# marco-wojtek/Exploring-MuZero-on-DOG

Hardware: AMD Instinct MI355X
Metric: self-play env steps/sec + MCTS sims/sec, det-MADN batch=4096, 1/2/4/8 GPU (higher is better)
Workload: dtype f32

## Files before the change

### exploring-muzero-on-dog_amd/csrc/launch.hpp

```cpp
#pragma once
#include "common.hpp"

namespace muz {

constexpr int kMaxSims = 100;
constexpr int kMaxNodes = kMaxSims + 1;
constexpr int kMaxDepth = 64;
static inline int check_search_limits(int num_simulations, int max_depth) {
  const bool ok = num_simulations >= 1 && num_simulations <= kMaxSims && max_depth >= 1 && max_depth <= kMaxDepth;
  return ok ? MUZ_OK : MUZ_E_UNSUPPORTED;
}
static inline int check_search_call(int num_simulations, int max_depth, int n, const void* root_logits,
                                    const void* root_value, const void* root_embedding, const void* legal_bits,
                                    const void* workspace, int64_t workspace_bytes, int64_t (*need)(int, int),
                                    const void* action, const void* action_weights, const void* root_value_out) {
  if (check_search_limits(num_simulations, max_depth)) return MUZ_E_UNSUPPORTED;
  MUZ_HOST_CHECK(n >= 0 && root_logits && root_value && root_embedding && legal_bits && workspace && action &&
                 action_weights && root_value_out);
  MUZ_HOST_CHECK(workspace_bytes >= need(n, num_simulations));
  return MUZ_OK;
}

static inline bool ring_scalar_base() {
  const char* e = getenv("MUZ_RING_ADDR");
  return !e || atoi(e) != 0;
}

struct SearchArgs {
  int S, D, max_considered;
  float value_scale, maxvisit_init, gumbel_scale;
  unsigned long long seed;
  int turn;
  const int32_t* key_game = nullptr;
  const int32_t* key_turn = nullptr;
  int exact_select = 0;
  int games_per_wg = 8;
};
static inline SearchArgs make_search_args(const muz_search_cfg& cfg) {
  SearchArgs sa;
  sa.S = cfg.num_simulations;
  sa.D = cfg.max_depth;
  sa.max_considered = cfg.max_num_considered;
  sa.value_scale = cfg.value_scale;
  sa.maxvisit_init = cfg.maxvisit_init;
  sa.gumbel_scale = cfg.gumbel_scale;
  sa.seed = cfg.seed;
  sa.turn = cfg.turn;
  return sa;
}

int launch_root_inference(const muz_net_w& w, const float* obs, int n, const int* n_dev, float* conv_scratch,
                          float* logits, float* value, float* emb, hipStream_t s, int32_t* host_counts = nullptr);

int launch_root_inference(const muz_classic_net_w& w, const float* obs, int n, const int* n_dev, float* conv_scratch,
                          float* logits, float* value, float* emb, hipStream_t s);

int launch_repr_conv(const muz_repr_w& r, const float* obs, int C, int n, const int* n_dev, float* conv,
                     hipStream_t s, int32_t* host_counts = nullptr);
int launch_dense0(const muz_dense& d0, int n, const int* n_dev, float* conv, hipStream_t s);
int launch_film(const muz_dyn_w& d, int A, hipStream_t s);

int launch_gumbel_search(const muz_net_w& w, const SearchArgs& sa, const float* root_logits, const float* root_value,
                         const float* root_emb, const uint32_t* legal, const float* gumbel, const int32_t* game_id,
                         int n, const int* n_dev, void* workspace, int32_t* action, float* weights, float* value,
                         hipStream_t s);

int64_t search_workspace_bytes(int n, int S);

struct PuctArgs {
  int S, D, qtransform;
  float min_value, max_value, dir_frac, dir_alpha, pb_c_init, pb_c_base, temperature;
  unsigned long long seed;
  int turn;
  const int32_t* key_game = nullptr;
  const int32_t* key_turn = nullptr;
};
template <class Cfg>
static inline PuctArgs puct_args_of(const Cfg& cfg, int qtransform, float min_value, float max_value) {
  PuctArgs pa;
  pa.S = cfg.num_simulations;
  pa.D = cfg.max_depth;
  pa.qtransform = qtransform;
  pa.min_value = min_value;
  pa.max_value = max_value;
  pa.dir_frac = cfg.dirichlet_fraction;
  pa.dir_alpha = cfg.dirichlet_alpha;
  pa.pb_c_init = cfg.pb_c_init;
  pa.pb_c_base = cfg.pb_c_base;
  pa.temperature = cfg.temperature;
  pa.seed = cfg.seed;
  pa.turn = cfg.turn;
  return pa;
}
static inline PuctArgs make_puct_args(const muz_puct_cfg& cfg) {
  return puct_args_of(cfg, cfg.qtransform, cfg.min_value, cfg.max_value);
}
static inline PuctArgs make_puct_args(const muz_stoch_cfg& cfg) {
  return puct_args_of(cfg, MUZ_QT_PARENT_SIBLINGS, -1.f, 1.f);
}
static inline int check_puct_cfg(const muz_puct_cfg& cfg) {
  if (cfg.qtransform != MUZ_QT_MIN_MAX && cfg.qtransform != MUZ_QT_PARENT_SIBLINGS) return MUZ_E_UNSUPPORTED;
  if (!(cfg.max_value > cfg.min_value)) return MUZ_E_UNSUPPORTED;
  if (!(cfg.dirichlet_fraction >= 0.f && cfg.dirichlet_fraction <= 1.f)) return MUZ_E_UNSUPPORTED;
  if (!(cfg.dirichlet_alpha > 0.f) || !(cfg.pb_c_base > 0.f) || !(cfg.temperature >= 0.f)) return MUZ_E_UNSUPPORTED;
  return MUZ_OK;
}
static inline int check_stoch_cfg(const muz_stoch_cfg& cfg) {
  if (!(cfg.dirichlet_fraction >= 0.f && cfg.dirichlet_fraction <= 1.f)) return MUZ_E_UNSUPPORTED;
  if (!(cfg.dirichlet_alpha > 0.f) || !(cfg.pb_c_base > 0.f) || !(cfg.temperature >= 0.f)) return MUZ_E_UNSUPPORTED;
  if (!(cfg.pb_c_init == cfg.pb_c_init)) return MUZ_E_UNSUPPORTED;
  return MUZ_OK;
}
int launch_puct_search(const muz_net_w& w, const PuctArgs& pa, const float* root_logits, const float* root_value,
                       const float* root_emb, const uint32_t* legal, const float* dirichlet, const float* gumbel,
                       const int32_t* game_id, int n, const int* n_dev, void* workspace, int32_t* action,
                       float* weights, float* value, hipStream_t s);

struct SArgs {
  int S, D, A;
  float dir_frac, dir_alpha, pb_c_init, pb_c_base, temperature;
  unsigned long long seed;
  int turn;
  const int32_t* key_game = nullptr;
  const int32_t* key_turn = nullptr;
};
SArgs make_sargs(const muz_stoch_cfg& cfg, int A);
int launch_stochastic_search(const muz_classic_net_w& w, const SArgs& sa, const float* root_logits,
                             const float* root_value, const float* root_emb, const uint32_t* legal,
                             const float* dirichlet, const float* gumbel, const int32_t* game_id, int n, const int* n_dev,
                             void* workspace, int32_t* action, float* weights, float* value, hipStream_t s);
int64_t stochastic_workspace_bytes(int n, int S);
int check_classic_net(const muz_classic_net_w* w);

}
```

### exploring-muzero-on-dog_amd/csrc/nets.hip

```cpp
#include <type_traits>

#include "launch.hpp"
#include "nn.hpp"

namespace muz {

constexpr int kConvRowsPad = 64;
constexpr int kPreLd = 64 + 4;
#ifndef MUZ_CONV_PAD
#define MUZ_CONV_PAD 8
#endif
constexpr int kC1Ld = 32 + MUZ_CONV_PAD;
constexpr int kC2Ld = 64 + MUZ_CONV_PAD;

template <int N, int LDO>
__device__ __forceinline__ void ln_positions(const float* pre, float* out, int out_row0, const AS4 muz_ln& P) {
  const int pos = threadIdx.x >> 2, q = threadIdx.x & 3;
  if (pos >= 56) return;
  constexpr int PER = N / 4;
  float v[PER], s = 0.f, s2 = 0.f;
#pragma unroll
  for (int i = 0; i < PER; ++i) {
    v[i] = pre[pos * kPreLd + q + 4 * i];
    s += v[i];
    s2 = fmaf(v[i], v[i], s2);
  }
  s += dpp<DPP_XOR1>(s);
  s += dpp<DPP_XOR2>(s);
  s2 += dpp<DPP_XOR1>(s2);
  s2 += dpp<DPP_XOR2>(s2);
  const float mean = s / (float)N, mean2 = s2 / (float)N;
  const float inv = ln_rstd(fmaxf(0.f, fmaf(-mean, mean, mean2)) + 1e-6f);
#pragma unroll
  for (int i = 0; i < PER; ++i) {
    const int c = q + 4 * i;
    out[(out_row0 + pos) * LDO + c] = fmaxf(fmaf(v[i] - mean, inv * gp(P.scale)[c], gp(P.bias)[c]), 0.f);
  }
}

template <int KB, int CIN, int LDI>
__device__ __forceinline__ void conv_mfma(const AS4 muz_dense& L, const float* in, float* pre) {
  static_assert(CIN % 16 == 0, "a k-block within one tap");
  const int lane = threadIdx.x & 63, wv = threadIdx.x >> 6;
  const int r = lane & 15, g = lane >> 4;
  const AS1 f32x4* wp = gp(reinterpret_cast<const f32x4*>(L.w)) + (size_t)wv * KB * 64 + lane;
  f32x4 acc[4];
#pragma unroll
  for (int t = 0; t < 4; ++t) acc[t] = f32x4{0.f, 0.f, 0.f, 0.f};
  f32x4 w0 = wp[0], w1 = KB > 1 ? wp[64] : w0, w2;
#pragma unroll
  for (int kb = 0; kb < KB; ++kb) {
    if (kb + 2 < KB) w2 = wp[(kb + 2) * 64];
    f32x4 a[4];
#pragma unroll
    for (int t = 0; t < 4; ++t)
      a[t] = *reinterpret_cast<const f32x4*>(in + (t * 16 + r + (kb * 16) / CIN) * LDI + (kb * 16) % CIN + 4 * g);
#pragma unroll
    for (int j = 0; j < 4; ++j)
#pragma unroll
      for (int t = 0; t < 4; ++t) acc[t] = mfma4(w0[j], a[t][j], acc[t]);
    w0 = w1;
    w1 = w2;
  }
  const AS1 f32x4* bias4 = gp(reinterpret_cast<const f32x4*>(L.b));
  const f32x4 bb = bias4[(16 * wv + 4 * g) >> 2];
#pragma unroll
  for (int t = 0; t < 4; ++t)
    *reinterpret_cast<f32x4*>(pre + (t * 16 + r) * kPreLd + 16 * wv + 4 * g) = acc[t] + bb;
}

__global__ __launch_bounds__(256) void k_repr_conv(muz_repr_w Rarg, const float* __restrict__ obs, int C, int n,
                                                   const int* __restrict__ n_dev, float* __restrict__ convout,
                                                   int32_t* host_counts) {
  if (host_counts && blockIdx.x == 0 && threadIdx.x == 0) {
    __hip_atomic_store(&host_counts[0], n_dev[0], __ATOMIC_RELAXED, __HIP_MEMORY_SCOPE_SYSTEM);
    __hip_atomic_store(&host_counts[1], n_dev[1], __ATOMIC_RELEASE, __HIP_MEMORY_SCOPE_SYSTEM);
  }
  if (n_dev) n = *n_dev;
  if ((int)blockIdx.x >= n) return;
  const AS4 muz_repr_w& R = *kernarg0<muz_repr_w>();
  __shared__ __attribute__((aligned(16))) float pre[kConvRowsPad * kPreLd];
  __shared__ __attribute__((aligned(16))) float buf[68 * kC2Ld];
  float* in0 = buf;
  float* c1in = buf + 352;
  float* c2in = buf;
  static_assert(352 >= 58 * 6 && 352 + 66 * kC1Ld <= 68 * kC2Ld, "conv LDS carve");
  const int g = blockIdx.x;
  const int tid = threadIdx.x;
  const float* o = obs + (size_t)g * C * 56;
  for (int i = tid; i < 58 * 6; i += 256) {
    const int w = i / 6 - 1, ch = i % 6;
    in0[i] = (w >= 0 && w < 56) ? o[ch * 56 + w] : 0.f;
  }
  for (int i = tid; i < 66 * kC1Ld; i += 256) c1in[i] = 0.f;
  __syncthreads();
  {
    const int co = tid & 31;
    float wk[18];
#pragma unroll
    for (int k = 0; k < 18; ++k) wk[k] = gp(R.conv0.w)[k * 32 + co];
    const float bco = gp(R.conv0.b)[co];
    for (int w = tid >> 5; w < 56; w += 8) {
      float s = 0.f;
#pragma unroll
      for (int k = 0; k < 18; ++k) s = fmaf(in0[w * 6 + k], wk[k], s);
      pre[w * kPreLd + co] = s + bco;
    }
  }
  __syncthreads();
  ln_positions<32, kC1Ld>(pre, c1in, 1, R.ln0);
  __syncthreads();
  conv_mfma<6, 32, kC1Ld>(R.conv1, c1in, pre);
  __syncthreads();
  for (int i = tid; i < 12 * kC2Ld; i += 256) c2in[(i < 2 * kC2Ld ? 0 : 56 * kC2Ld) + i] = 0.f;
  ln_positions<64, kC2Ld>(pre, c2in, 2, R.ln1);
  __syncthreads();
  conv_mfma<20, 64, kC2Ld>(R.conv2, c2in, pre);
  __syncthreads();
  ln_positions<64, 64>(pre, c2in, 0, R.ln2);
  __syncthreads();
  float* dst = convout + (size_t)g * kConvRowFloats;
  for (int i = tid; i < kConvMapFloats; i += 256) dst[i] = c2in[i];
}

#ifndef MUZ_CONV_PAIR
#define MUZ_CONV_PAIR 3
#endif
constexpr int kPairThreads = MUZ_CONV_PAIR == 2 ? 512 : 256;
constexpr int kPairRows = 112, kPairTiles = 7;
constexpr int kG0 = 58, kG1 = 58, kG2 = 60;

template <int N, int LDO, int GR, int PAD>
__device__ __forceinline__ void ln_pair(const float* pre, float* out, const AS4 muz_ln& P) {
  const int q = threadIdx.x & 3;
  constexpr int PER = N / 4;
#pragma unroll
  for (int pass = 0; pass < 512 / kPairThreads; ++pass) {
    const int pos = (threadIdx.x >> 2) + (kPairThreads / 4) * pass;
    if (pos >= kPairRows) break;
    float v[PER], s = 0.f, s2 = 0.f;
#pragma unroll
    for (int i = 0; i < PER; ++i) {
      v[i] = pre[pos * kPreLd + q + 4 * i];
      s += v[i];
      s2 = fmaf(v[i], v[i], s2);
    }
    s += dpp<DPP_XOR1>(s);
    s += dpp<DPP_XOR2>(s);
    s2 += dpp<DPP_XOR1>(s2);
    s2 += dpp<DPP_XOR2>(s2);
    const float mean = s / (float)N, mean2 = s2 / (float)N;
    const float inv = ln_rstd(fmaxf(0.f, fmaf(-mean, mean, mean2)) + 1e-6f);
    const int gm = pos >= 56 ? 1 : 0, orow = gm * GR + PAD + pos - 56 * gm;
#pragma unroll
    for (int i = 0; i < PER; ++i) {
      const int c = q + 4 * i;
      out[orow * LDO + c] = fmaxf(fmaf(v[i] - mean, inv * gp(P.scale)[c], gp(P.bias)[c]), 0.f);
    }
  }
}

template <int KB, int CIN, int LDI, int GR, int T0, int NT>
__device__ __forceinline__ void conv_mfma_pair(const AS4 muz_dense& L, const float* in, float* pre) {
  static_assert(CIN % 16 == 0, "a k-block within one tap");
  const int lane = threadIdx.x & 63, wv = (threadIdx.x >> 6) & 3;
  const int r = lane & 15, g = lane >> 4;
  const AS1 f32x4* wp = gp(reinterpret_cast<const f32x4*>(L.w)) + (size_t)wv * KB * 64 + lane;
  int roff[NT];
#pragma unroll
  for (int t = 0; t < NT; ++t) {
    const int R = (T0 + t) * 16 + r, gm = R >= 56 ? 1 : 0;
    roff[t] = (gm * GR + R - 56 * gm) * LDI + 4 * g;
  }
  f32x4 acc[NT];
#pragma unroll
  for (int t = 0; t < NT; ++t) acc[t] = f32x4{0.f, 0.f, 0.f, 0.f};
  f32x4 w0 = wp[0], w1 = KB > 1 ? wp[64] : w0, w2;
#pragma unroll
  for (int kb = 0; kb < KB; ++kb) {
    if (kb + 2 < KB) w2 = wp[(kb + 2) * 64];
    f32x4 a[NT];
#pragma unroll
    for (int t = 0; t < NT; ++t)
      a[t] = *reinterpret_cast<const f32x4*>(in + roff[t] + ((kb * 16) / CIN) * LDI + (kb * 16) % CIN);
#pragma unroll
    for (int j = 0; j < 4; ++j)
#pragma unroll
      for (int t = 0; t < NT; ++t) acc[t] = mfma4(w0[j], a[t][j], acc[t]);
    w0 = w1;
    w1 = w2;
  }
  const AS1 f32x4* bias4 = gp(reinterpret_cast<const f32x4*>(L.b));
  const f32x4 bb = bias4[(16 * wv + 4 * g) >> 2];
#pragma unroll
  for (int t = 0; t < NT; ++t)
    *reinterpret_cast<f32x4*>(pre + ((T0 + t) * 16 + r) * kPreLd + 16 * wv + 4 * g) = acc[t] + bb;
}

template <int KB, int CIN, int LDI, int GR>
__device__ __forceinline__ void conv_pair(const AS4 muz_dense& L, const float* in, float* pre) {
  if (kPairThreads == 256)
    conv_mfma_pair<KB, CIN, LDI, GR, 0, kPairTiles>(L, in, pre);
  else if (threadIdx.x < 256)
    conv_mfma_pair<KB, CIN, LDI, GR, 0, 4>(L, in, pre);
  else
    conv_mfma_pair<KB, CIN, LDI, GR, 4, 3>(L, in, pre);
}

__global__ __launch_bounds__(kPairThreads) void k_repr_conv2(muz_repr_w Rarg, const float* __restrict__ obs, int C, int n,
                                                    const int* __restrict__ n_dev, float* __restrict__ convout,
                                                    int32_t* host_counts) {
  if (host_counts && blockIdx.x == 0 && threadIdx.x == 0) {
    __hip_atomic_store(&host_counts[0], n_dev[0], __ATOMIC_RELAXED, __HIP_MEMORY_SCOPE_SYSTEM);
    __hip_atomic_store(&host_counts[1], n_dev[1], __ATOMIC_RELEASE, __HIP_MEMORY_SCOPE_SYSTEM);
  }
  if (n_dev) n = *n_dev;
  const int g0 = 2 * (int)blockIdx.x;
  if (g0 >= n) return;
  const int ng = g0 + 1 < n ? 2 : 1;
  const AS4 muz_repr_w& R = *kernarg0<muz_repr_w>();
  __shared__ __attribute__((aligned(16))) float pre[kPairRows * kPreLd];
  __shared__ __attribute__((aligned(16))) float buf[2 * kG2 * kC2Ld];
  float* in0 = buf;
  float* c1in = buf + 704;
  float* c2in = buf;
  static_assert(704 >= 2 * kG0 * 6 && 704 + 2 * kG1 * kC1Ld <= 2 * kG2 * kC2Ld && kPairRows * 64 <= 2 * kG2 * kC2Ld,
                "pair conv LDS carve");
  const int tid = threadIdx.x;
  for (int i = tid; i < 2 * kG0 * 6; i += kPairThreads) {
    const int gm = i / (kG0 * 6), j = i % (kG0 * 6), w = j / 6 - 1, ch = j % 6;
    in0[i] = (gm < ng && w >= 0 && w < 56) ? obs[((size_t)(g0 + gm) * C + ch) * 56 + w] : 0.f;
  }
  for (int i = tid; i < 2 * kG1 * kC1Ld; i += kPairThreads) c1in[i] = 0.f;
  __syncthreads();
  {
    const int co = tid & 31;
    float wk[18];
#pragma unroll
    for (int k = 0; k < 18; ++k) wk[k] = gp(R.conv0.w)[k * 32 + co];
    const float bco = gp(R.conv0.b)[co];
    for (int p = tid >> 5; p < kPairRows; p += kPairThreads / 32) {
      const int gm = p >= 56 ? 1 : 0;
      const float* x = in0 + gm * kG0 * 6 + (p - 56 * gm) * 6;
      float s = 0.f;
#pragma unroll
      for (int k = 0; k < 18; ++k) s = fmaf(x[k], wk[k], s);
      pre[p * kPreLd + co] = s + bco;
    }
  }
  __syncthreads();
  ln_pair<32, kC1Ld, kG1, 1>(pre, c1in, R.ln0);
  __syncthreads();
  conv_pair<6, 32, kC1Ld, kG1>(R.conv1, c1in, pre);
  __syncthreads();
  for (int i = tid; i < 8 * kC2Ld; i += kPairThreads) {
    const int rr = i / kC2Ld, row = (rr >> 2) * kG2 + ((rr & 3) < 2 ? (rr & 3) : 56 + (rr & 3));
    c2in[row * kC2Ld + i % kC2Ld] = 0.f;
  }
  ln_pair<64, kC2Ld, kG2, 2>(pre, c2in, R.ln1);
  __syncthreads();
  conv_pair<20, 64, kC2Ld, kG2>(R.conv2, c2in, pre);
  __syncthreads();
  ln_pair<64, 64, 56, 0>(pre, c2in, R.ln2);
  __syncthreads();
  for (int i = tid; i < ng * kConvMapFloats; i += kPairThreads) {
    const int gm = i >= kConvMapFloats ? 1 : 0;
    convout[(size_t)(g0 + gm) * kConvRowFloats + i - gm * kConvMapFloats] = c2in[i];
  }
}

constexpr int kC1Ld3 = 36, kC2Ld3 = 68, kP0Ld = 36;
constexpr int kIn0F = 704, kPre0At = kIn0F, kC1At = kPre0At + kPairRows * kP0Ld, kStatAt = kC1At + 2 * kG1 * kC1Ld3;
constexpr int kConv3Floats = kStatAt + kPairRows * 8;
static_assert(2 * kG0 * 6 <= kIn0F && 2 * kG2 * kC2Ld3 <= kStatAt && kConv3Floats * 4 <= 40 * 1024, "conv3 LDS carve");

template <int N, int LDI, int LDO, int GR, int PAD>
__device__ __forceinline__ void ln_pair_ld(const float* pre, float* out, const AS4 muz_ln& P) {
  const int q = threadIdx.x & 3;
  constexpr int PER = N / 4;
#pragma unroll
  for (int pass = 0; pass < 2; ++pass) {
    const int pos = (threadIdx.x >> 2) + 64 * pass;
    if (pos >= kPairRows) break;
    float v[PER], s = 0.f, s2 = 0.f;
#pragma unroll
    for (int i = 0; i < PER; ++i) {
      v[i] = pre[pos * LDI + q + 4 * i];
      s += v[i];
      s2 = fmaf(v[i], v[i], s2);
    }
    s += dpp<DPP_XOR1>(s);
    s += dpp<DPP_XOR2>(s);
    s2 += dpp<DPP_XOR1>(s2);
    s2 += dpp<DPP_XOR2>(s2);
    const float mean = s / (float)N, mean2 = s2 / (float)N;
    const float inv = ln_rstd(fmaxf(0.f, fmaf(-mean, mean, mean2)) + 1e-6f);
    const int gm = pos >= 56 ? 1 : 0, orow = gm * GR + PAD + pos - 56 * gm;
#pragma unroll
    for (int i = 0; i < PER; ++i) {
      const int c = q + 4 * i;
      out[orow * LDO + c] = fmaxf(fmaf(v[i] - mean, inv * gp(P.scale)[c], gp(P.bias)[c]), 0.f);
    }
  }
}

template <int KB, int CIN, int LDI, int GR>
__device__ __forceinline__ void conv_acc_pair(const AS4 muz_dense& L, const float* in, f32x4 (&acc)[kPairTiles],
                                              float* st) {
  static_assert(CIN % 16 == 0, "a k-block within one tap");
  const int lane = threadIdx.x & 63, wv = threadIdx.x >> 6;
  const int r = lane & 15, g = lane >> 4;
  const AS1 f32x4* wp = gp(reinterpret_cast<const f32x4*>(L.w)) + (size_t)wv * KB * 64 + lane;
  int roff[kPairTiles];
#pragma unroll
  for (int t = 0; t < kPairTiles; ++t) {
    const int R = t * 16 + r, gm = R >= 56 ? 1 : 0;
    roff[t] = (gm * GR + R - 56 * gm) * LDI + 4 * g;
    acc[t] = f32x4{0.f, 0.f, 0.f, 0.f};
  }
  f32x4 w0 = wp[0], w1 = KB > 1 ? wp[64] : w0, w2;
#pragma unroll
  for (int kb = 0; kb < KB; ++kb) {
    if (kb + 2 < KB) w2 = wp[(kb + 2) * 64];
    f32x4 a[kPairTiles];
#pragma unroll
    for (int t = 0; t < kPairTiles; ++t)
      a[t] = *reinterpret_cast<const f32x4*>(in + roff[t] + ((kb * 16) / CIN) * LDI + (kb * 16) % CIN);
#pragma unroll
    for (int j = 0; j < 4; ++j)
#pragma unroll
      for (int t = 0; t < kPairTiles; ++t) acc[t] = mfma4(w0[j], a[t][j], acc[t]);
    w0 = w1;
    w1 = w2;
  }
  const f32x4 bb = gp(reinterpret_cast<const f32x4*>(L.b))[(16 * wv + 4 * g) >> 2];
#pragma unroll
  for (int t = 0; t < kPairTiles; ++t) {
    acc[t] += bb;
    float s = (acc[t][0] + acc[t][1]) + (acc[t][2] + acc[t][3]);
    float s2 = fmaf(acc[t][3], acc[t][3], fmaf(acc[t][2], acc[t][2], fmaf(acc[t][1], acc[t][1], acc[t][0] * acc[t][0])));
    LoHi<float> p = swap16(s);
    s = p.lo + p.hi;
    p = swap16(s2);
    s2 = p.lo + p.hi;
    p = swap32(s);
    s = p.lo + p.hi;
    p = swap32(s2);
    s2 = p.lo + p.hi;
    if (g == 0) *reinterpret_cast<float2*>(st + (t * 16 + r) * 8 + 2 * wv) = make_float2(s, s2);
  }
}

template <class F>
__device__ __forceinline__ void ln_acc_pair(const f32x4 (&acc)[kPairTiles], const float* st, const AS4 muz_ln& P,
                                            F out) {
  const int lane = threadIdx.x & 63, wv = threadIdx.x >> 6;
  const int r = lane & 15, g = lane >> 4, c0 = 16 * wv + 4 * g;
  const f32x4 ga = gp(reinterpret_cast<const f32x4*>(P.scale))[c0 >> 2];
  const f32x4 be = gp(reinterpret_cast<const f32x4*>(P.bias))[c0 >> 2];
#pragma unroll
  for (int t = 0; t < kPairTiles; ++t) {
    const int pos = t * 16 + r;
    const f32x4 a = *reinterpret_cast<const f32x4*>(st + pos * 8);
    const f32x4 b = *reinterpret_cast<const f32x4*>(st + pos * 8 + 4);
    const float s = ((a[0] + a[2]) + b[0]) + b[2], s2 = ((a[1] + a[3]) + b[1]) + b[3];
    const float mean = s / 64.f, mean2 = s2 / 64.f;
    const float inv = ln_rstd(fmaxf(0.f, fmaf(-mean, mean, mean2)) + 1e-6f);
    f32x4 o;
#pragma unroll
    for (int j = 0; j < 4; ++j) o[j] = fmaxf(fmaf(acc[t][j] - mean, inv * ga[j], be[j]), 0.f);
    out(pos, c0, o);
  }
}

__global__ __launch_bounds__(256) void k_repr_conv3(muz_repr_w Rarg, const float* __restrict__ obs, int C, int n,
                                                    const int* __restrict__ n_dev, float* __restrict__ convout,
                                                    int32_t* host_counts) {
  if (host_counts && blockIdx.x == 0 && threadIdx.x == 0) {
    __hip_atomic_store(&host_counts[0], n_dev[0], __ATOMIC_RELAXED, __HIP_MEMORY_SCOPE_SYSTEM);
    __hip_atomic_store(&host_counts[1], n_dev[1], __ATOMIC_RELEASE, __HIP_MEMORY_SCOPE_SYSTEM);
  }
  if (n_dev) n = *n_dev;
  const int g0 = 2 * (int)blockIdx.x;
  if (g0 >= n) return;
  const int ng = g0 + 1 < n ? 2 : 1;
  const AS4 muz_repr_w& R = *kernarg0<muz_repr_w>();
  __shared__ __attribute__((aligned(16))) float sm[kConv3Floats];
  float* in0 = sm;
  float* pre0 = sm + kPre0At;
  float* c1in = sm + kC1At;
  float* c2in = sm;
  float* st = sm + kStatAt;
  const int tid = threadIdx.x;
  for (int i = tid; i < 2 * kG0 * 6; i += 256) {
    const int gm = i / (kG0 * 6), j = i % (kG0 * 6), w = j / 6 - 1, ch = j % 6;
    in0[i] = (gm < ng && w >= 0 && w < 56) ? obs[((size_t)(g0 + gm) * C + ch) * 56 + w] : 0.f;
  }
  for (int i = tid; i < 4 * kC1Ld3; i += 256) {
    const int rr = i / kC1Ld3;
    c1in[((rr >> 1) * kG1 + (rr & 1) * 57) * kC1Ld3 + i % kC1Ld3] = 0.f;
  }
  __syncthreads();
  {
    const int co = tid & 31;
    float wk[18];
#pragma unroll
    for (int k = 0; k < 18; ++k) wk[k] = gp(R.conv0.w)[k * 32 + co];
    const float bco = gp(R.conv0.b)[co];
    for (int p = tid >> 5; p < kPairRows; p += 8) {
      const int gm = p >= 56 ? 1 : 0;
      const float* x = in0 + gm * kG0 * 6 + (p - 56 * gm) * 6;
      float s = 0.f;
#pragma unroll
      for (int k = 0; k < 18; ++k) s = fmaf(x[k], wk[k], s);
      pre0[p * kP0Ld + co] = s + bco;
    }
  }
  __syncthreads();
  ln_pair_ld<32, kP0Ld, kC1Ld3, kG1, 1>(pre0, c1in, R.ln0);
  __syncthreads();
  f32x4 acc[kPairTiles];
  conv_acc_pair<6, 32, kC1Ld3, kG1>(R.conv1, c1in, acc, st);
  __syncthreads();
  for (int i = tid; i < 8 * kC2Ld3; i += 256) {
    const int rr = i / kC2Ld3, row = (rr >> 2) * kG2 + ((rr & 3) < 2 ? (rr & 3) : 56 + (rr & 3));
    c2in[row * kC2Ld3 + i % kC2Ld3] = 0.f;
  }
  ln_acc_pair(acc, st, R.ln1, [&](int pos, int c0, const f32x4& o) {
    const int gm = pos >= 56 ? 1 : 0;
    *reinterpret_cast<f32x4*>(c2in + (gm * kG2 + 2 + pos - 56 * gm) * kC2Ld3 + c0) = o;
  });
  __syncthreads();
  conv_acc_pair<20, 64, kC2Ld3, kG2>(R.conv2, c2in, acc, st);
  __syncthreads();
  ln_acc_pair(acc, st, R.ln2, [&](int pos, int c0, const f32x4& o) {
    const int gm = pos >= 56 ? 1 : 0;
    if (gm < ng)
      *reinterpret_cast<f32x4*>(convout + (size_t)(g0 + gm) * kConvRowFloats + (pos - 56 * gm) * 64 + c0) = o;
  });
}

#ifndef MUZ_D0_NG
#define MUZ_D0_NG 2
#endif
#ifndef MUZ_D0_KC
#define MUZ_D0_KC 4
#endif
constexpr int kD0Rows = 64, kD0NG = MUZ_D0_NG, kD0KC = MUZ_D0_KC, kD0Ld = kD0KC * 16 + 8;
constexpr int kD0KB = kConvMapFloats / 16, kD0Chunks = kD0KB / kD0KC;
constexpr int kD0CB = 8 / kD0NG;
constexpr int kD0AF4 = kD0Rows * kD0KC * 4;
constexpr int kD0WF4 = kD0NG * kD0KC * 128;
static_assert(kD0KB % kD0KC == 0 && (kD0NG == 1 || kD0NG == 2), "Dense_0 chunks");
static_assert(kD0AF4 % 512 == 0 && kD0WF4 % 512 == 0, "Dense_0 staging: whole float4 per thread");

__global__ __launch_bounds__(512) void k_dense0(muz_dense d0, int n, const int* __restrict__ n_dev, float* conv) {
  if (n_dev) n = *n_dev;
  const int id = blockIdx.x, slot = id >> 3;
  const int rb = (slot / kD0CB) * 8 + (id & 7), cb = slot % kD0CB;
  const int row0 = rb * kD0Rows;
  if (row0 >= n) return;
  __shared__ __attribute__((aligned(16))) float sA[2][kD0Rows * kD0Ld];
  __shared__ f32x4 sW[2][kD0WF4];
  const int t = threadIdx.x, lane = t & 63, wv = t >> 6;
  constexpr int TW = kD0NG;
  const int rt = wv & 3, part = wv >> 2, r = lane & 15, g = lane >> 4;
  constexpr int kGroupF4 = kD0KB * 64 * 2;
  const AS1 f32x4* Wg = gp(reinterpret_cast<const f32x4*>(d0.w)) + (size_t)(kD0NG * cb) * kGroupF4;
  constexpr int QA = kD0AF4 / 512, QW = kD0WF4 / 512;
  f32x4 ra[QA], rw[QW];
  auto gload = [&](int c) {
#pragma unroll
    for (int q = 0; q < QA; ++q) {
      const int i = t + 512 * q;
      const int row = row0 + i / (4 * kD0KC);
      ra[q] = row < n ? *gp(reinterpret_cast<const f32x4*>(conv + (size_t)row * kConvRowFloats + c * 16 * kD0KC) +
                            i % (4 * kD0KC))
                      : f32x4{0.f, 0.f, 0.f, 0.f};
    }
#pragma unroll
    for (int q = 0; q < QW; ++q) {
      const int i = t + 512 * q;
      rw[q] = Wg[(size_t)(i / (kD0KC * 128)) * kGroupF4 + c * (kD0KC * 128) + i % (kD0KC * 128)];
    }
  };
  auto lstore = [&](int b) {
#pragma unroll
    for (int q = 0; q < QA; ++q) {
      const int i = t + 512 * q;
      *reinterpret_cast<f32x4*>(&sA[b][(i / (4 * kD0KC)) * kD0Ld + 4 * (i % (4 * kD0KC))]) = ra[q];
    }
#pragma unroll
    for (int q = 0; q < QW; ++q) {
      const int i = t + 512 * q;
      const int j = i % (kD0KC * 128), kb = j >> 7, ln = (j >> 1) & 63, tt = j & 1;
      sW[b][(i / (kD0KC * 128)) * (kD0KC * 128) + (kb * 2 + tt) * 64 + ln] = rw[q];
    }
  };
  f32x4 acc[TW];
#pragma unroll
  for (int tt = 0; tt < TW; ++tt) acc[tt] = f32x4{0.f, 0.f, 0.f, 0.f};
  constexpr int kPer = kD0Chunks / kD0KSplit;
  static_assert(kD0Chunks % kD0KSplit == 0, "Dense_0 k split");
  const int cbeg = (int)blockIdx.y * kPer;
  gload(cbeg);
  lstore(0);
  __syncthreads();
#pragma unroll 1
  for (int c = 0; c < kPer; ++c) {
    const int b = c & 1;
    if (c + 1 < kPer) gload(cbeg + c + 1);
#pragma unroll
    for (int kb = 0; kb < kD0KC; ++kb) {
      const f32x4 a = *reinterpret_cast<const f32x4*>(&sA[b][(rt * 16 + r) * kD0Ld + kb * 16 + 4 * g]);
      f32x4 w[TW];
#pragma unroll
      for (int tt = 0; tt < TW; ++tt) {
        const int grp = kD0NG == 2 ? part : 0, tile = kD0NG == 2 ? tt : part;
        w[tt] = sW[b][grp * (kD0KC * 128) + (kb * 2 + tile) * 64 + lane];
      }
#pragma unroll
      for (int j = 0; j < 4; ++j)
#pragma unroll
        for (int tt = 0; tt < TW; ++tt) acc[tt] = mfma4(w[tt][j], a[j], acc[tt]);
    }
    if (c + 1 < kPer) lstore(b ^ 1);
    __syncthreads();
  }
  const int row = row0 + rt * 16 + r;
  if (row < n) {
    const AS1 f32x4* bias4 = gp(reinterpret_cast<const f32x4*>(d0.b));
#pragma unroll
    for (int tt = 0; tt < TW; ++tt) {
      const int col = kD0NG == 2 ? (2 * cb + part) * 32 + tt * 16 + 4 * g : cb * 32 + part * 16 + 4 * g;
      float* dst = conv + (size_t)row * kConvRowFloats + kConvMapFloats + 256 * blockIdx.y + col;
      *reinterpret_cast<f32x4*>(dst) = kD0KSplit > 1 ? acc[tt] : acc[tt] + bias4[col >> 2];
    }
  }
}

int launch_dense0(const muz_dense& d0, int n, const int* n_dev, float* conv, hipStream_t s) {
  const int rbs = (n + kD0Rows - 1) / kD0Rows;
  const int wgs = (rbs + 7) / 8 * 8 * kD0CB;
  k_dense0<<<dim3(wgs, kD0KSplit), 512, 0, s>>>(d0, n, n_dev, conv);
  return muz_last_launch_error();
}

template <class NW, bool SB>
__global__ __launch_bounds__(kThreads) void k_root_dense(NW Wt, const float* __restrict__ obs,
                                                    const float* __restrict__ convout, int n,
                                                    const int* __restrict__ n_dev, float* prior_logits, float* value,
                                                    float* embedding) {
  if (n_dev) n = *n_dev;
  if ((int)blockIdx.x * kRows >= n) return;
  __shared__ __attribute__((aligned(16))) float smem[kArenaFloats];
  const Arena a = Arena::carve(smem);
  const AS4 NW* W = kernarg0<NW>();
  const int A = Wt.num_actions;
  const int g0 = blockIdx.x * kRows;
  const int row = trow(), sub = tsub();
  const int gr = g0 + row;
  const bool valid = gr < n;
  PfT<SB> pf;
  repr16<NT256, true>(W->repr, obs, Wt.obs_channels, convout, g0, n, a, pf, &W->pred.rb[0].d0, LAT, LAT);
  __syncthreads();
  minmax16(a.T, LD);
  __syncthreads();
  if (valid)
    for (int c = sub; c < LAT; c += kRowLanes) embedding[(size_t)gr * LAT + c] = a.T[row * LD + c];
  __syncthreads();
  pred16<1, false, false, kSplitkLogits && std::is_same<NW, muz_net_w>::value>(W->pred, A, a.T, a, pf, nullptr, 0, 0);
  if (valid) {
    for (int c = sub; c < A; c += kRowLanes) prior_logits[(size_t)gr * A + c] = a.U[row * LD + c];
    if (sub == 0) value[gr] = a.v0[row];
  }
}

template <bool SB>
__global__ __launch_bounds__(kThreads) void k_recurrent(muz_net_w Wt, const int32_t* __restrict__ action,
                                                   const float* __restrict__ emb, int n, float* reward,
                                                   float* discount, float* prior_logits, float* value,
                                                   float* next_emb) {
  __shared__ __attribute__((aligned(16))) float smem[kArenaFloats];
  const Arena a = Arena::carve(smem);
  const int A = Wt.num_actions;
  const int g0 = blockIdx.x * kRows;
  const int row = trow(), sub = tsub();
  const int gr = g0 + row;
  const bool valid = gr < n;
  const AS4 muz_net_w* W = kernarg0<muz_net_w>();
  const int ar = valid ? action[gr] : 0;
  const DynIn din = dyn_load(W->dyn, A, valid ? gp(emb) + (size_t)gr * LAT : nullptr, ar);
  PfT<SB> pf;
  pf_issue<NT256>(pf, &W->dyn.d3, LAT, LAT);
  dyn16<NT256>(W->dyn, A, din, ar, a, pf, &W->pred.rb[0].d0, LAT, LAT);
  if (valid) {
    for (int c = sub; c < LAT; c += kRowLanes) next_emb[(size_t)gr * LAT + c] = a.T[row * LD + c];
    if (sub == 0) {
      reward[gr] = a.v1[row];
      discount[gr] = a.v2[row];
    }
  }
  pred16<1, false, false, kSplitkLogits>(W->pred, A, a.T, a, pf, nullptr, 0, 0);
  if (valid) {
    for (int c = sub; c < A; c += kRowLanes) prior_logits[(size_t)gr * A + c] = a.U[row * LD + c];
    if (sub == 0) value[gr] = a.v0[row];
  }
}

__global__ __launch_bounds__(512) void k_film(muz_dyn_w D, int A) {
  __shared__ float e[64];
  const int a = blockIdx.x, n = threadIdx.x;
  if (n < 64) e[n] = fmaxf((a < A ? D.d0.w[a * 64 + n] : 0.f) + D.d0.b[n], 0.f);
  __syncthreads();
  const int w = (n >> 4) / NT512, t = (n >> 4) % NT512;
  float acc = 0.f;
  for (int k = 0; k < 64; ++k) {
    const int kb = k >> 4, lane = ((k & 15) >> 2) * 16 + (n & 15), j = k & 3;
    acc = fmaf(e[k], D.d12.w[((((size_t)w * 4 + kb) * 64 + lane) * NT512 + t) * 4 + j], acc);
  }
  D.film[a * 512 + n] = acc + D.d12.b[n];
}

int check_net(const muz_net_w* w) {
  if (!w) return MUZ_E_INVALID;
  if (!w->dyn.film) return MUZ_E_INVALID;
  if (w->num_actions != MUZ_DET_ACTIONS) return MUZ_E_UNSUPPORTED;
  if (w->obs_channels < 7 || w->obs_channels > 38) return MUZ_E_UNSUPPORTED;
  return MUZ_OK;
}

int launch_repr_conv(const muz_repr_w& r, const float* obs, int C, int n, const int* n_dev, float* conv,
                     hipStream_t s, int32_t* host_counts) {
  if (host_counts && !n_dev) return MUZ_E_INVALID;
  if (MUZ_CONV_PAIR == 3)
    k_repr_conv3<<<(n + 1) / 2, 256, 0, s>>>(r, obs, C, n, n_dev, conv, host_counts);
  else if (MUZ_CONV_PAIR)
    k_repr_conv2<<<(n + 1) / 2, kPairThreads, 0, s>>>(r, obs, C, n, n_dev, conv, host_counts);
  else
    k_repr_conv<<<n, 256, 0, s>>>(r, obs, C, n, n_dev, conv, host_counts);
  return muz_last_launch_error();
}

int launch_film(const muz_dyn_w& d, int A, hipStream_t s) {
  k_film<<<A + 1, 512, 0, s>>>(d, A);
  return muz_last_launch_error();
}

template <class NW>
static int launch_root_impl(const NW& w, const float* obs, int n, const int* n_dev, float* conv, float* logits,
                            float* value, float* emb, hipStream_t s, int32_t* host_counts = nullptr) {
  int rc = launch_repr_conv(w.repr, obs, w.obs_channels, n, n_dev, conv, s, host_counts);
  if (rc) return rc;
  rc = launch_dense0(w.repr.d0, n, n_dev, conv, s);
  if (rc) return rc;
  if (ring_scalar_base())
    k_root_dense<NW, true><<<(n + kRows - 1) / kRows, kThreads, 0, s>>>(w, obs, conv, n, n_dev, logits, value, emb);
  else
    k_root_dense<NW, false><<<(n + kRows - 1) / kRows, kThreads, 0, s>>>(w, obs, conv, n, n_dev, logits, value, emb);
  return muz_last_launch_error();
}

int launch_root_inference(const muz_net_w& w, const float* obs, int n, const int* n_dev, float* conv, float* logits,
                          float* value, float* emb, hipStream_t s, int32_t* host_counts) {
  return launch_root_impl(w, obs, n, n_dev, conv, logits, value, emb, s, host_counts);
}

int launch_root_inference(const muz_classic_net_w& w, const float* obs, int n, const int* n_dev, float* conv,
                          float* logits, float* value, float* emb, hipStream_t s) {
  return launch_root_impl(w, obs, n, n_dev, conv, logits, value, emb, s);
}

}

using namespace muz;

extern "C" {

int32_t muz_tile_waves(void) { return kWaves; }

int muz_net_prepare(const muz_net_w* w, void* stream) {
  if (!w || !w->dyn.film || !w->dyn.d0.w || !w->dyn.d0.b || !w->dyn.d12.w || !w->dyn.d12.b) return MUZ_E_INVALID;
  if (w->num_actions != MUZ_DET_ACTIONS) return MUZ_E_UNSUPPORTED;
  k_film<<<w->num_actions + 1, 512, 0, (hipStream_t)stream>>>(w->dyn, w->num_actions);
  return muz_last_launch_error();
}

int64_t muz_nets_root_scratch_bytes(int32_t n) {
  const int64_t rows = ((int64_t)n + kRows - 1) / kRows * kRows;
  return rows * kConvRowFloats * (int64_t)sizeof(float);
}

int muz_nets_root(const muz_net_w* w, const float* obs, int32_t n, void* scratch, int64_t scratch_bytes,
                  float* prior_logits, float* value, float* embedding, void* stream) {
  int rc = check_net(w);
  if (rc) return rc;
  MUZ_HOST_CHECK(n >= 0 && obs && scratch && prior_logits && value && embedding);
  MUZ_HOST_CHECK(scratch_bytes >= muz_nets_root_scratch_bytes(n));
  if (n == 0) return MUZ_OK;
  return launch_root_inference(*w, obs, n, nullptr, (float*)scratch, prior_logits, value, embedding,
                               (hipStream_t)stream);
}

int muz_nets_recurrent(const muz_net_w* w, const int32_t* action, const float* embedding, int32_t n, float* reward,
                       float* discount, float* prior_logits, float* value, float* next_embedding, void* stream) {
  int rc = check_net(w);
  if (rc) return rc;
  MUZ_HOST_CHECK(n >= 0 && action && embedding && reward && discount && prior_logits && value && next_embedding);
  if (n == 0) return MUZ_OK;
  if (ring_scalar_base())
    k_recurrent<true><<<(n + kRows - 1) / kRows, kThreads, 0, (hipStream_t)stream>>>(
        *w, action, embedding, n, reward, discount, prior_logits, value, next_embedding);
  else
    k_recurrent<false><<<(n + kRows - 1) / kRows, kThreads, 0, (hipStream_t)stream>>>(
        *w, action, embedding, n, reward, discount, prior_logits, value, next_embedding);
  return muz_last_launch_error();
}

}
```

Measured before the change: 1.085 million.

## Software-pipeline root conv and dense0 loads, move conv0 onto MFMA

Adds an env-selected new form of the root representation network, on by default. conv_acc_pair and k_dense0 double-buffer their LDS operand loads one k-block ahead, with sched barriers, so reads overlap the MFMAs. dense0 also issues the global loads two chunks ahead and writes LDS earlier, or spreads those writes across k-blocks in form 2. The first conv layer moves from scalar FMAs to an MFMA-based routine. The extra buffers raise register pressure, and the scheduling gains cover only the root inference part of self-play.

```diff
diff --git a/exploring-muzero-on-dog_amd/csrc/launch.hpp b/exploring-muzero-on-dog_amd/csrc/launch.hpp
--- a/exploring-muzero-on-dog_amd/csrc/launch.hpp
+++ b/exploring-muzero-on-dog_amd/csrc/launch.hpp
@@ -24,6 +24,15 @@
 static inline bool ring_scalar_base() {
   const char* e = getenv("MUZ_RING_ADDR");
   return !e || atoi(e) != 0;
+}
+
+static inline bool root_form_new() {
+  const char* e = getenv("MUZ_ROOT_FORM");
+  return !e || atoi(e) != 0;
+}
+static inline int root_dev() {
+  const char* e = getenv("MUZ_ROOT_DEV");
+  return e ? atoi(e) : 0;
 }
 
 struct SearchArgs {
diff --git a/exploring-muzero-on-dog_amd/csrc/nets.hip b/exploring-muzero-on-dog_amd/csrc/nets.hip
--- a/exploring-muzero-on-dog_amd/csrc/nets.hip
+++ b/exploring-muzero-on-dog_amd/csrc/nets.hip
@@ -304,7 +304,7 @@
   }
 }
 
-template <int KB, int CIN, int LDI, int GR>
+template <int KB, int CIN, int LDI, int GR, bool PIPE>
 __device__ __forceinline__ void conv_acc_pair(const AS4 muz_dense& L, const float* in, f32x4 (&acc)[kPairTiles],
                                               float* st) {
   static_assert(CIN % 16 == 0, "a k-block within one tap");
@@ -319,17 +319,24 @@
     acc[t] = f32x4{0.f, 0.f, 0.f, 0.f};
   }
   f32x4 w0 = wp[0], w1 = KB > 1 ? wp[64] : w0, w2;
+  f32x4 a[2][kPairTiles];
+  auto lda = [&](int kb, f32x4 (&d)[kPairTiles]) {
+#pragma unroll
+    for (int t = 0; t < kPairTiles; ++t)
+      d[t] = *reinterpret_cast<const f32x4*>(in + roff[t] + ((kb * 16) / CIN) * LDI + (kb * 16) % CIN);
+  };
+  if (PIPE) lda(0, a[0]);
 #pragma unroll
   for (int kb = 0; kb < KB; ++kb) {
     if (kb + 2 < KB) w2 = wp[(kb + 2) * 64];
-    f32x4 a[kPairTiles];
-#pragma unroll
-    for (int t = 0; t < kPairTiles; ++t)
-      a[t] = *reinterpret_cast<const f32x4*>(in + roff[t] + ((kb * 16) / CIN) * LDI + (kb * 16) % CIN);
+    if (!PIPE) lda(kb, a[kb & 1]);
+    else if (kb + 1 < KB) lda(kb + 1, a[(kb + 1) & 1]);
+    if (PIPE) __builtin_amdgcn_sched_barrier(0);
 #pragma unroll
     for (int j = 0; j < 4; ++j)
 #pragma unroll
-      for (int t = 0; t < kPairTiles; ++t) acc[t] = mfma4(w0[j], a[t][j], acc[t]);
+      for (int t = 0; t < kPairTiles; ++t) acc[t] = mfma4(w0[j], a[kb & 1][t][j], acc[t]);
+    if (PIPE) __builtin_amdgcn_sched_barrier(0);
     w0 = w1;
     w1 = w2;
   }
@@ -373,6 +380,33 @@
   }
 }
 
+__device__ __forceinline__ void conv0_mfma_pair(const AS4 muz_dense& L, const float* in0, float* pre0) {
+  const int lane = threadIdx.x & 63, wv = threadIdx.x >> 6;
+  const int r = lane & 15, g = lane >> 4, ct = wv & 1, t0 = wv >> 1;
+  float w[5];
+#pragma unroll
+  for (int s = 0; s < 5; ++s) w[s] = 4 * s + g < 18 ? gp(L.w)[(4 * s + g) * 32 + 16 * ct + r] : 0.f;
+  const f32x4 bb = gp(reinterpret_cast<const f32x4*>(L.b))[(16 * ct + 4 * g) >> 2];
+  f32x4 acc[4];
+  const float* x[4];
+#pragma unroll
+  for (int i = 0; i < 4; ++i) {
+    const int t = t0 + 2 * i < kPairTiles ? t0 + 2 * i : t0;
+    const int R = t * 16 + r, gm = R >= 56 ? 1 : 0;
+    x[i] = in0 + gm * kG0 * 6 + (R - 56 * gm) * 6 + g;
+    acc[i] = f32x4{0.f, 0.f, 0.f, 0.f};
+  }
+#pragma unroll
+  for (int s = 0; s < 5; ++s)
+#pragma unroll
+    for (int i = 0; i < 4; ++i) acc[i] = mfma4(w[s], 4 * s + g < 18 ? x[i][4 * s] : 0.f, acc[i]);
+#pragma unroll
+  for (int i = 0; i < 4; ++i)
+    if (t0 + 2 * i < kPairTiles)
+      *reinterpret_cast<f32x4*>(pre0 + ((t0 + 2 * i) * 16 + r) * kP0Ld + 16 * ct + 4 * g) = acc[i] + bb;
+}
+
+template <bool NEW>
 __global__ __launch_bounds__(256) void k_repr_conv3(muz_repr_w Rarg, const float* __restrict__ obs, int C, int n,
                                                     const int* __restrict__ n_dev, float* __restrict__ convout,
                                                     int32_t* host_counts) {
@@ -401,7 +435,9 @@
     c1in[((rr >> 1) * kG1 + (rr & 1) * 57) * kC1Ld3 + i % kC1Ld3] = 0.f;
   }
   __syncthreads();
-  {
+  if (NEW) {
+    conv0_mfma_pair(R.conv0, in0, pre0);
+  } else {
     const int co = tid & 31;
     float wk[18];
 #pragma unroll
@@ -420,7 +456,7 @@
   ln_pair_ld<32, kP0Ld, kC1Ld3, kG1, 1>(pre0, c1in, R.ln0);
   __syncthreads();
   f32x4 acc[kPairTiles];
-  conv_acc_pair<6, 32, kC1Ld3, kG1>(R.conv1, c1in, acc, st);
+  conv_acc_pair<6, 32, kC1Ld3, kG1, NEW>(R.conv1, c1in, acc, st);
   __syncthreads();
   for (int i = tid; i < 8 * kC2Ld3; i += 256) {
     const int rr = i / kC2Ld3, row = (rr >> 2) * kG2 + ((rr & 3) < 2 ? (rr & 3) : 56 + (rr & 3));
@@ -431,7 +467,7 @@
     *reinterpret_cast<f32x4*>(c2in + (gm * kG2 + 2 + pos - 56 * gm) * kC2Ld3 + c0) = o;
   });
   __syncthreads();
-  conv_acc_pair<20, 64, kC2Ld3, kG2>(R.conv2, c2in, acc, st);
+  conv_acc_pair<20, 64, kC2Ld3, kG2, NEW>(R.conv2, c2in, acc, st);
   __syncthreads();
   ln_acc_pair(acc, st, R.ln2, [&](int pos, int c0, const f32x4& o) {
     const int gm = pos >= 56 ? 1 : 0;
@@ -454,7 +490,9 @@
 static_assert(kD0KB % kD0KC == 0 && (kD0NG == 1 || kD0NG == 2), "Dense_0 chunks");
 static_assert(kD0AF4 % 512 == 0 && kD0WF4 % 512 == 0, "Dense_0 staging: whole float4 per thread");
 
+template <int FORM>
 __global__ __launch_bounds__(512) void k_dense0(muz_dense d0, int n, const int* __restrict__ n_dev, float* conv) {
+  constexpr bool WAB = FORM > 0, PIPE = FORM > 0, RBW = FORM == 1, SPREAD = FORM == 2;
   if (n_dev) n = *n_dev;
   const int id = blockIdx.x, slot = id >> 3;
   const int rb = (slot / kD0CB) * 8 + (id & 7), cb = slot % kD0CB;
@@ -484,18 +522,20 @@
       rw[q] = Wg[(size_t)(i / (kD0KC * 128)) * kGroupF4 + c * (kD0KC * 128) + i % (kD0KC * 128)];
     }
   };
+  auto lstore_a = [&](int b, int q) {
+    const int i = t + 512 * q;
+    *reinterpret_cast<f32x4*>(&sA[b][(i / (4 * kD0KC)) * kD0Ld + 4 * (i % (4 * kD0KC))]) = ra[q];
+  };
+  auto lstore_w = [&](int b, int q) {
+    const int i = t + 512 * q;
+    const int j = i % (kD0KC * 128), kb = j >> 7, ln = (j >> 1) & 63, tt = j & 1;
+    sW[b][(i / (kD0KC * 128)) * (kD0KC * 128) + (kb * 2 + tt) * 64 + ln] = rw[q];
+  };
   auto lstore = [&](int b) {
 #pragma unroll
-    for (int q = 0; q < QA; ++q) {
-      const int i = t + 512 * q;
-      *reinterpret_cast<f32x4*>(&sA[b][(i / (4 * kD0KC)) * kD0Ld + 4 * (i % (4 * kD0KC))]) = ra[q];
-    }
-#pragma unroll
-    for (int q = 0; q < QW; ++q) {
-      const int i = t + 512 * q;
-      const int j = i % (kD0KC * 128), kb = j >> 7, ln = (j >> 1) & 63, tt = j & 1;
-      sW[b][(i / (kD0KC * 128)) * (kD0KC * 128) + (kb * 2 + tt) * 64 + ln] = rw[q];
-    }
+    for (int q = 0; q < QA; ++q) lstore_a(b, q);
+#pragma unroll
+    for (int q = 0; q < QW; ++q) lstore_w(b, q);
   };
   f32x4 acc[TW];
 #pragma unroll
@@ -505,26 +545,51 @@
   const int cbeg = (int)blockIdx.y * kPer;
   gload(cbeg);
   lstore(0);
+  if (WAB && kPer > 1) gload(cbeg + 1);
   __syncthreads();
 #pragma unroll 1
   for (int c = 0; c < kPer; ++c) {
     const int b = c & 1;
-    if (c + 1 < kPer) gload(cbeg + c + 1);
-#pragma unroll
-    for (int kb = 0; kb < kD0KC; ++kb) {
-      const f32x4 a = *reinterpret_cast<const f32x4*>(&sA[b][(rt * 16 + r) * kD0Ld + kb * 16 + 4 * g]);
-      f32x4 w[TW];
+    f32x4 a[2], w[2][TW];
+    auto ldf = [&](int kb, f32x4& a_, f32x4 (&w_)[TW]) {
+      a_ = *reinterpret_cast<const f32x4*>(&sA[b][(rt * 16 + r) * kD0Ld + kb * 16 + 4 * g]);
 #pragma unroll
       for (int tt = 0; tt < TW; ++tt) {
         const int grp = kD0NG == 2 ? part : 0, tile = kD0NG == 2 ? tt : part;
-        w[tt] = sW[b][grp * (kD0KC * 128) + (kb * 2 + tile) * 64 + lane];
+        w_[tt] = sW[b][grp * (kD0KC * 128) + (kb * 2 + tile) * 64 + lane];
       }
+    };
+    if (RBW) {
+      ldf(0, a[0], w[0]);
+      __builtin_amdgcn_sched_barrier(0);
+    }
+    static_assert(!SPREAD || (WAB && PIPE && !RBW && QA + QW == kD0KC), "one staged float4 per k-block");
+    if (SPREAD) {
+    } else if (WAB) {
+      if (c + 1 < kPer) lstore(b ^ 1);
+      if (c + 2 < kPer) gload(cbeg + c + 2);
+    } else if (c + 1 < kPer) {
+      gload(cbeg + c + 1);
+    }
+    if (PIPE && !RBW) ldf(0, a[0], w[0]);
+#pragma unroll
+    for (int kb = 0; kb < kD0KC; ++kb) {
+      if (!PIPE) ldf(kb, a[kb & 1], w[kb & 1]);
+      else if (kb + 1 < kD0KC) ldf(kb + 1, a[(kb + 1) & 1], w[(kb + 1) & 1]);
+      if (SPREAD && c + 1 < kPer) {
+        if (kb < QA) lstore_a(b ^ 1, kb);
+        else lstore_w(b ^ 1, kb - QA);
+      }
+      if (PIPE) __builtin_amdgcn_sched_barrier(0);
 #pragma unroll
       for (int j = 0; j < 4; ++j)
 #pragma unroll
-        for (int tt = 0; tt < TW; ++tt) acc[tt] = mfma4(w[tt][j], a[j], acc[tt]);
-    }
-    if (c + 1 < kPer) lstore(b ^ 1);
+        for (int tt = 0; tt < TW; ++tt)
+          acc[tt] = mfma4(w[kb & 1][tt][j], a[kb & 1][j], acc[tt]);
+      if (PIPE) __builtin_amdgcn_sched_barrier(0);
+    }
+    if (!WAB && c + 1 < kPer) lstore(b ^ 1);
+    if (SPREAD && c + 2 < kPer) gload(cbeg + c + 2);
     __syncthreads();
   }
   const int row = row0 + rt * 16 + r;
@@ -542,7 +607,12 @@
 int launch_dense0(const muz_dense& d0, int n, const int* n_dev, float* conv, hipStream_t s) {
   const int rbs = (n + kD0Rows - 1) / kD0Rows;
   const int wgs = (rbs + 7) / 8 * 8 * kD0CB;
-  k_dense0<<<dim3(wgs, kD0KSplit), 512, 0, s>>>(d0, n, n_dev, conv);
+  const dim3 grid(wgs, kD0KSplit);
+  switch (!root_form_new() ? 0 : root_dev() == 2 ? 2 : 1) {
+    case 0: k_dense0<0><<<grid, 512, 0, s>>>(d0, n, n_dev, conv); break;
+    case 1: k_dense0<1><<<grid, 512, 0, s>>>(d0, n, n_dev, conv); break;
+    default: k_dense0<2><<<grid, 512, 0, s>>>(d0, n, n_dev, conv); break;
+  }
   return muz_last_launch_error();
 }
 
@@ -633,9 +703,12 @@
 int launch_repr_conv(const muz_repr_w& r, const float* obs, int C, int n, const int* n_dev, float* conv,
                      hipStream_t s, int32_t* host_counts) {
   if (host_counts && !n_dev) return MUZ_E_INVALID;
-  if (MUZ_CONV_PAIR == 3)
-    k_repr_conv3<<<(n + 1) / 2, 256, 0, s>>>(r, obs, C, n, n_dev, conv, host_counts);
-  else if (MUZ_CONV_PAIR)
+  if (MUZ_CONV_PAIR == 3) {
+    if (root_form_new())
+      k_repr_conv3<true><<<(n + 1) / 2, 256, 0, s>>>(r, obs, C, n, n_dev, conv, host_counts);
+    else
+      k_repr_conv3<false><<<(n + 1) / 2, 256, 0, s>>>(r, obs, C, n, n_dev, conv, host_counts);
+  } else if (MUZ_CONV_PAIR)
     k_repr_conv2<<<(n + 1) / 2, kPairThreads, 0, s>>>(r, obs, C, n, n_dev, conv, host_counts);
   else
     k_repr_conv<<<n, 256, 0, s>>>(r, obs, C, n, n_dev, conv, host_counts);
```

Result: no change. 1.087 million, median of 6 (+0.2%).
